# TravisWheelerLab/BATH

Hardware: AMD Instinct MI355X
Metric: DP Gcells/s + residues/s through bathsearch pipeline at 1/2/4/8 MI355X (higher is better)
Workload: dtype u8/i16 integer scores (SSV: exact binary16), f32 Forward

## Files before the change

### bath_amd/csrc/bath_kernels.hpp

```cpp
#pragma once
#include <climits>
#include <hip/hip_runtime.h>

#include <cstdint>

#include "bath_common.hpp"
#include "bath_hip.h"

namespace bath {

typedef short s16x2 __attribute__((ext_vector_type(2)));

template <int CTRL, int ROW_MASK = 0xf>
__device__ __forceinline__ int dpp_i(int v, int old) { return __builtin_amdgcn_update_dpp(old, v, CTRL, ROW_MASK, 0xf, false); }
__device__ __forceinline__ int wave_shr1_i32(int v, int fill) { return dpp_i<0x138>(v, fill); }
__device__ __forceinline__ float wave_shr1_f32(float v, float fill) {
  return __builtin_bit_cast(float, __builtin_amdgcn_update_dpp(__builtin_bit_cast(int, fill), __builtin_bit_cast(int, v), 0x138, 0xf, 0xf, false));
}
__device__ __forceinline__ float wave_max_f32(float v) {
  const int ninf = (int)0xff800000;
#define BATH_FMAX_STEP(CTRL, MASK) v = fmaxf(v, __builtin_bit_cast(float, __builtin_amdgcn_update_dpp(ninf, __builtin_bit_cast(int, v), CTRL, MASK, 0xf, false)));
  BATH_FMAX_STEP(0x111, 0xf) BATH_FMAX_STEP(0x112, 0xf) BATH_FMAX_STEP(0x114, 0xf) BATH_FMAX_STEP(0x118, 0xf) BATH_FMAX_STEP(0x142, 0xa) BATH_FMAX_STEP(0x143, 0xc)
#undef BATH_FMAX_STEP
  return __builtin_bit_cast(float, __builtin_amdgcn_readlane(__builtin_bit_cast(int, v), 63));
// ... 158 lines not shown
    const s16x2 xBv = __builtin_bit_cast(s16x2, bh);
    const s16x2 wrap = __builtin_bit_cast(s16x2, __builtin_amdgcn_alignbit(__builtin_bit_cast(unsigned, reg[NR - 1]), 0u, 16));
    s16x2 xE = zero, xE2 = zero;
#pragma unroll
    for (int g = NR / 4 - 1; g >= 0; g--) {
      const ssv_i4 inc = row[g];
      const int r = 4 * g;
      const s16x2 v3 = ssv_add(msv_pkmax(reg[r + 2], xBv), inc.w);
      const s16x2 v2 = ssv_add(msv_pkmax(reg[r + 1], xBv), inc.z);
      const s16x2 v1 = ssv_add(msv_pkmax(reg[r], xBv), inc.y);
      const s16x2 v0 = ssv_add(msv_pkmax((r > 0) ? reg[r - 1] : wrap, xBv), inc.x);
      reg[r + 3] = v3; reg[r + 2] = v2; reg[r + 1] = v1; reg[r] = v0;
      xE = ssv_max3(xE, v3, v2);
      xE2 = ssv_max3(xE2, v1, v0);
    }
    const h16x2 e1 = __builtin_bit_cast(h16x2, xE), e2 = __builtin_bit_cast(h16x2, xE2);
    int xEi = (int)(fmaxf(fmaxf((float)e1.x, (float)e1.y), fmaxf((float)e2.x, (float)e2.y)) * 2048.0f);
    if (xEi + c.bias >= 255) over = true;
    xEi = max(xEi - c.tec, 0);
    xJ = max(xJ, xEi);
    xB = max(max(c.base, xJ) - tjbm, 0);
  }
  *overflow = over;
  return xJ;
}
__device__ __forceinline__ float msv_lane_score(int xJ, int tjb, const MsvConsts &c) {
  float r = ((float)(xJ - tjb) - (float)c.base);
  r /= c.scale_b;
  return (float)((double)r - 3.0);
}

struct WindowRec { int32_t cand, n, k, length; float score; };

__device__ __forceinline__ float bias_forward(const uint8_t *s, int L, int M, const float *e , float p1) {
  const float L1 = (float)M / 8.0f;
  const float t00 = p1, t01 = 1.0f - p1, t10 = 1.0f / (L1 + 1.0f), t11 = L1 / (L1 + 1.0f);
  float logsc = 0.0f;
  if (L <= 0) return logsc;
  int x = min((int)s[0], 28);
  float d0 = e[2 * x] * 0.999f, d1 = e[2 * x + 1] * 0.001f;
  float mx = fmaxf(fmaxf(d0, 0.0f), d1);
  d0 /= mx; d1 /= mx;
  logsc += (float)log((double)mx);
  auto step = [&](int xx) {
    float n0 = 0.0f + d0 * t00; n0 = n0 + d1 * t10; n0 *= e[2 * xx];
    float n1 = 0.0f + d0 * t01; n1 = n1 + d1 * t11; n1 *= e[2 * xx + 1];
    mx = fmaxf(fmaxf(n0, 0.0f), n1);
    d0 = n0 / mx; d1 = n1 / mx;
    logsc += (float)log((double)mx);
  };
  int i = 1;
  uint32_t wnext = (i + 4 <= L) ? *reinterpret_cast<const uint32_t *>(s + i) : 0u;
  for (; i + 4 <= L; i += 4) {
    const uint32_t w = wnext;
    if (i + 8 <= L) wnext = *reinterpret_cast<const uint32_t *>(s + i + 4);
#pragma unroll
    for (int j = 0; j < 4; j++) step(min((int)((w >> (8 * j)) & 0xffu), 28));
  }
  for (; i < L; i++) step(min((int)s[i], 28));
  float end = 0.0f + d0 * 1.0f; end = end + d1 * 1.0f;
  logsc += (float)log((double)end);
  return logsc;
}

}
```

### bath_amd/csrc/bath_pipeline.hip

```cpp
#include <algorithm>
#include <cmath>
#include <cstring>
#include <cstdlib>
#include <map>
#include <thread>

#include "bath_common.hpp"
#include "bath_kernels.hpp"
#include "bath_launch.hpp"
#include "host_model.hpp"

using namespace bath;

namespace bath {

static const double kLog2 = 0.69314718055994529;

enum { FLAG_VIT_RUN = 1, FLAG_HAS_WIN = 2 };

struct Counters {
  int cand_count, todo_msv, todo_vit, todo_ssvb, todo_vit2, todo_fwd, win_count, overflow;
  int todo_lb, pad_;
  unsigned long long n_orfs, orf_res;
  unsigned long long n_past_msv, n_past_bias, n_past_vit, n_past_fwd;
// ... 295 lines not shown
  for (int k = k_start; k <= k_end; k++) {
    const float lo = ((float)base_b - (float)ssv_scores[(size_t)k * kKp + x]) / scale_b;
    acc += bgf[x] * expf(lo);
  }
  return acc;
}
__device__ void local_compo_finish(float *compo , const float *bgf, float *eo );
__device__ void local_compo_eo(const uint8_t *ssv_scores, int M, int base_b, float scale_b, const float *bgf, int k_start, int k_end, float *eo ) {
  float compo[20];
  for (int x = 0; x < 20; x++) compo[x] = local_compo_x(ssv_scores, M, base_b, scale_b, bgf, k_start, k_end, x);
  local_compo_finish(compo, bgf, eo);
}
__device__ void local_compo_finish(float *compo, const float *bgf, float *eo) {
  float sum = 0.f, cc = 0.f;
  for (int x = 0; x < 20; x++) { const float y = compo[x] - cc; const float t = sum + y; cc = (t - sum) - y; sum = t; }
  if (sum != 0.0f) for (int x = 0; x < 20; x++) compo[x] /= sum;
  else for (int x = 0; x < 20; x++) compo[x] = 1.0f / 20.0f;
  for (int x = 0; x < 20; x++) { eo[2 * x] = bgf[x] / bgf[x]; eo[2 * x + 1] = compo[x] / bgf[x]; }
  eo[2 * 20] = eo[2 * 20 + 1] = 1.0f; eo[2 * 27] = eo[2 * 27 + 1] = 1.0f; eo[2 * 28] = eo[2 * 28 + 1] = 1.0f;
  const int mem[6][2] = {{2, 11}, {7, 9}, {3, 13}, {8, 8}, {1, 1}, {-1, -1}};
  for (int dx = 0; dx < 6; dx++) {
    float n0 = 0.f, n1 = 0.f, den = 0.f;
    if (dx == 5) { for (int y = 0; y < 20; y++) { n0 += bgf[y]; n1 += compo[y]; den += bgf[y]; } }
    else {
      const int a = min(mem[dx][0], mem[dx][1]), b = max(mem[dx][0], mem[dx][1]);
      n0 += bgf[a]; n1 += compo[a]; den += bgf[a];
      if (b != a) { n0 += bgf[b]; n1 += compo[b]; den += bgf[b]; }
    }
    eo[2 * (21 + dx)] = den > 0.f ? n0 / den : 0.f;
    eo[2 * (21 + dx) + 1] = den > 0.f ? n1 / den : 0.f;
  }
}

__global__ void post_vit_kernel(Cand cand, int cand_cap, Counters *__restrict__ ctr, Params p, int32_t *__restrict__ todo_lb, int32_t *__restrict__ todo_fwd) {
  const int ncand = min(ctr->cand_count, cand_cap);
  for (int c = blockIdx.x * blockDim.x + threadIdx.x; c < ncand; c += gridDim.x * blockDim.x) {
    if (cand.stage[c] != 2) continue;
    const int L = cand.len[c];
    if (cand.flags[c] & FLAG_VIT_RUN) {
      const float seqsc = (float)((double)(cand.vfsc[c] - cand.filtersc[c]) / kLog2);
      const double P = d_gumbel_surv(seqsc, p.evparam[2], p.evparam[3]);
      cand.P[c] = P;
      if (P > p.F2) { cand.kminmax[2 * c] = 1 << 30; cand.kminmax[2 * c + 1] = 0; continue; }
    }
    atomicAdd(&ctr->n_past_vit, 1ull); atomicAdd(&ctr->pos_past_vit, (unsigned long long)L * 3ull);
    if (p.do_bias && cand.kminmax[2 * c] <= cand.kminmax[2 * c + 1]) {
      cand.flags[c] |= FLAG_HAS_WIN;
      todo_lb[atomicAdd(&ctr->todo_lb, 1)] = c;
      continue;
    }
    cand.stage[c] = 3;
    todo_fwd[atomicAdd(&ctr->todo_fwd, 1)] = c; atomicAdd(&ctr->res_fwd, (unsigned long long)L);
  }
}

__global__ void compo_terms_kernel(const float *__restrict__ bgf, int base_b, float scale_b, float *__restrict__ terms ) {
  const int x = blockIdx.x, sc = threadIdx.x;
  const float lo = ((float)base_b - (float)sc) / scale_b;
  terms[x * 256 + sc] = bgf[x] * expf(lo);
}

__global__ __launch_bounds__(64) void local_compo_kernel(Cand cand, const Counters *__restrict__ ctr, int M, const uint8_t *__restrict__ ssv_scores,
                                                         const float *__restrict__ terms, const int32_t *__restrict__ todo_lb, float *__restrict__ compo_out ) {
  const int lane = threadIdx.x, g = lane / 20, x = lane % 20;
  const int ntodo = ctr->todo_lb;
  for (int base = blockIdx.x * 3; base < ntodo; base += gridDim.x * 3) {
    const int job = base + g;
    if (g >= 3 || job >= ntodo) continue;
    const int c = todo_lb[job];
    int k_start = cand.kminmax[2 * c], k_end = cand.kminmax[2 * c + 1];
    const int k_len = k_end - k_start + 1;
    if (k_len < 20) { k_start -= (20 - k_len) / 2; k_end += (20 - k_len) / 2; }
    k_start = max(1, k_start); k_end = min(M, k_end);
    const float *tx = terms + x * 256;
    float acc = 0.0f;
    for (int k = k_start; k <= k_end; k++) acc += tx[ssv_scores[(size_t)k * kKp + x]];
    compo_out[(size_t)job * 20 + x] = acc;
  }
}

__global__ __launch_bounds__(64) void post_vit_local_kernel(Cand cand, Counters *__restrict__ ctr, Params p, const uint8_t *__restrict__ pool, int M,
                                                            const float *__restrict__ bgf, const float *__restrict__ compo_in,
                                                            const float *__restrict__ p1_tab, const float *__restrict__ lt1_tab, const float *__restrict__ lt2_tab,
                                                            const int32_t *__restrict__ todo_lb, int32_t *__restrict__ todo_vit2, int32_t *__restrict__ todo_fwd) {
  __shared__ float s_eo[64][kKp * 2 + 1];
  const int ntodo = ctr->todo_lb;
  for (int job = blockIdx.x * blockDim.x + threadIdx.x; job < ntodo; job += gridDim.x * blockDim.x) {
    const int c = todo_lb[job];
    const int L = cand.len[c];
    const float usc = cand.usc[c];
    float filtersc = cand.filtersc[c];
    const float vfsc = (cand.flags[c] & FLAG_VIT_RUN) ? cand.vfsc[c] : -INFINITY;
    float compo[20];
    for (int y = 0; y < 20; y++) compo[y] = compo_in[(size_t)job * 20 + y];
    float *eo = s_eo[threadIdx.x];
    local_compo_finish(compo, bgf, eo);
    float lf = bias_forward(pool + cand.off[c], L, M, eo, p1_tab[L]);
    lf = (lf + lt1_tab[L]) + lt2_tab[L];
    bool to_fwd = true;
    if (lf > filtersc) {
      filtersc = lf;
      cand.filtersc[c] = filtersc;
      if (vfsc == -INFINITY) {
        const float seqsc = (float)((double)(usc - filtersc) / kLog2);
        const double P = d_gumbel_surv(seqsc, p.evparam[0], p.evparam[1]);
        cand.P[c] = P;
        if (P > p.F2) { cand.stage[c] = 5; todo_vit2[atomicAdd(&ctr->todo_vit2, 1)] = c; atomicAdd(&ctr->res_vit, (unsigned long long)L); to_fwd = false; }
      } else {
        const float seqsc = (float)((double)(vfsc - filtersc) / kLog2);
        const double P = d_gumbel_surv(seqsc, p.evparam[2], p.evparam[3]);
        cand.P[c] = P;
        if (P > p.F2) to_fwd = false;
      }
    }
    if (to_fwd) { cand.stage[c] = 3; todo_fwd[atomicAdd(&ctr->todo_fwd, 1)] = c; atomicAdd(&ctr->res_fwd, (unsigned long long)L); }
  }
}

__global__ void post_vit2_kernel(Cand cand, Counters *__restrict__ ctr, Params p, const int32_t *__restrict__ todo_vit2, int32_t *__restrict__ todo_fwd) {
  const int ntodo = ctr->todo_vit2;
  for (int job = blockIdx.x * blockDim.x + threadIdx.x; job < ntodo; job += gridDim.x * blockDim.x) {
    const int c = todo_vit2[job];
    const float seqsc = (float)((double)(cand.vfsc[c] - cand.filtersc[c]) / kLog2);
    const double P = d_gumbel_surv(seqsc, p.evparam[2], p.evparam[3]);
    cand.P[c] = P;
    if (P > p.F2) { cand.stage[c] = 2; continue; }
    cand.stage[c] = 3;
    todo_fwd[atomicAdd(&ctr->todo_fwd, 1)] = c; atomicAdd(&ctr->res_fwd, (unsigned long long)cand.len[c]);
  }
}

__global__ void final_kernel(Cand cand, Counters *__restrict__ ctr, Params p, const int32_t *__restrict__ todo_fwd) {
  const int ntodo = ctr->todo_fwd;
  for (int job = blockIdx.x * blockDim.x + threadIdx.x; job < ntodo; job += gridDim.x * blockDim.x) {
    const int c = todo_fwd[job];
    const float seqsc = (float)((double)(cand.fwdsc[c] - cand.filtersc[c]) / kLog2);
    const double P = d_exp_surv(seqsc, p.evparam[4], p.evparam[5]);
    cand.P[c] = P;
    if (P > (p.fs_pipe ? p.F4 : p.F3)) continue;
    cand.stage[c] = 4;
    atomicAdd(&ctr->n_past_fwd, 1ull);
    if (!p.fs_pipe) atomicAdd(&ctr->pos_past_fwd, (unsigned long long)cand.len[c] * 3ull);
  }
}

__global__ void copy_count_kernel(const int *src, int64_t *dst) { *dst = *src; }

}
// ... 133 lines not shown
}

static int cascade_model_ok(bath_hip_ctx *ctx, const bath_hip_oprofile *om) {
  if (om->M <= kCascadeMaxNodes) return BATH_OK;
  ctx->set_error("the filter cascade supports models up to " + std::to_string(kCascadeMaxNodes) + " nodes (this one has " + std::to_string(om->M) + ")");
  return BATH_EINVAL;
}

static int launch_ssv_bath(bath_hip_ctx *ctx, hipStream_t stream, const bath_hip_oprofile *om, const Cand &cand, Counters *ctr, const int32_t *todo, const uint8_t *pool,
                           const uint8_t *ssv_scores, const MsvConsts &mc, double invP, WindowRec *wins, int win_cap);

static int run_filters(bath_hip_ctx *ctx, const bath_hip_oprofile *om, const bath_hip_seqs *dna,
                       const bath_pipeline_params *prm, bath_pipeline_stats *stats,
                       const bath_orf_result **results, int64_t *n_results, FilterState *state) {
  if (!ctx || !om || !dna || !prm) return BATH_EINVAL;
  if (cascade_model_ok(ctx, om) != BATH_OK) return BATH_EINVAL;
  BATH_HIP_TRY(ctx, hipSetDevice(ctx->device));
  if (n_results) *n_results = 0;
  if (results) *results = nullptr;
  if (stats) std::memset(stats, 0, sizeof *stats);
  const int64_t nwin = dna->n;
  if (nwin == 0) return BATH_OK;
  const int M = om->M;
  const int max_orf = dna->maxlen / 3 + 1;
  int st = om->ensure_len_tables(max_orf);
  if (st != BATH_OK) return st;

  OrfTablesDev tt{};
  if (prm->strands < 0 || prm->strands > 2 || prm->initiator < 0 || prm->initiator > 2) { ctx->set_error("bath_pipeline_params: strands / initiator out of range"); return BATH_EINVAL; }
  if ((st = orf_tables_upload(ctx, prm->ncbi_table, &tt, prm->initiator)) != BATH_OK) return st;
  if ((st = ensure_emit_table(ctx, om, prm->F1, max_orf)) != BATH_OK) return st;
  DevBuf &b_tabs = ctx->scratch[8], &b_work = ctx->scratch[9];
  const size_t ssv_bytes = (size_t)(M + 1) * kKp;
  const size_t tabs_bytes = 8192 + ssv_bytes + 256 + 20 * 4 + 256;
  if (tabs_bytes > b_tabs.cap) ctx->tabs_uid = 0;
  BATH_HIP_TRY(ctx, b_tabs.reserve(tabs_bytes));
  char *tp = b_tabs.as<char>();
  const int16_t *d_emit = om->d_emit;
  uint8_t *d_ssvsc = reinterpret_cast<uint8_t *>(tp); tp += (ssv_bytes + 255) / 256 * 256;
  float *d_bgf = reinterpret_cast<float *>(tp);
  if (ctx->tabs_uid != om->uid || ctx->tabs_ptr != b_tabs.p) {
    std::vector<uint8_t> ssv_scores(ssv_bytes, 0);
    bath_hip_oprofile_get_ssv_scores(om, ssv_scores.data());
    BATH_HIP_TRY(ctx, hipMemcpyAsync(d_ssvsc, ssv_scores.data(), ssv_scores.size(), hipMemcpyHostToDevice, ctx->stream));
    BATH_HIP_TRY(ctx, hipMemcpyAsync(d_bgf, kAminoBg, 20 * sizeof(float), hipMemcpyHostToDevice, ctx->stream));
    BATH_HIP_TRY(ctx, hipStreamSynchronize(ctx->stream));
    ctx->tabs_uid = om->uid; ctx->tabs_ptr = b_tabs.p;
  }

  Params P{};
  P.F1 = prm->F1; P.F2 = prm->F2; P.F3 = prm->F3; P.F4 = prm->F4;
  P.do_bias = prm->do_biasfilter; P.fs_pipe = prm->fs_pipe; P.minlen = prm->min_orf_len;
  std::memcpy(P.evparam, om->evparam, sizeof P.evparam);
  const MsvConsts mc = msv_consts(om);
  const double invP_f1 = gumbel_invsurv(prm->F1, om->evparam[0], om->evparam[1]);
  VitWindowArgs wa{};
  wa.invP_vit = (double)(float)gumbel_invsurv(prm->F2, om->evparam[2], om->evparam[3]);
  wa.invP_msv = (double)(float)gumbel_invsurv(prm->F2, om->evparam[0], om->evparam[1]);

  if (dna->cache_minlen != prm->min_orf_len) {
    int64_t nres_c = 0, max_orfs_c = 0;
    for (int64_t i = 0; i < nwin; i++) {
      const int n = dna->h_len[i];
      if (n < 15) continue;
      nres_c += 2 * (int64_t)(n - (dna->h_context.empty() ? 0 : dna->h_context[(size_t)i]));
      max_orfs_c += 6 * (int64_t)((n / 3 + 1) / (prm->min_orf_len + 1) + 1);
    }
    dna->cache_minlen = prm->min_orf_len; dna->cache_nres = nres_c; dna->cache_max_orfs = max_orfs_c;
  }
  const int64_t nres = prm->strands == BATH_STRAND_BOTH ? dna->cache_nres : dna->cache_nres / 2;
  const int64_t max_orfs = dna->cache_max_orfs;
  if (max_orfs >= (int64_t)INT32_MAX) { ctx->set_error("DNA block too large for one pipeline call (ORF list indices are 32-bit): split it"); return BATH_EINVAL; }
  int64_t cap = std::max<int64_t>(4096, (int64_t)((double)max_orfs * std::min(1.0, prm->F1 * 4.0 + 0.01)));
  cap = std::min<int64_t>(cap, std::max<int64_t>(max_orfs, 4096));

  if ((st = orf_tiles_ensure(ctx, dna)) != BATH_OK) return st;
  const size_t nent = (size_t)dna->ntiles * 6;
  DevBuf &b_aa = ctx->scratch[24], &b_slots = ctx->scratch[25], &b_orfs = ctx->scratch[26], &b_misc = ctx->scratch[27];
// ... 64 lines not shown
                       om->ssv_row_bytes, om->lt.d_tjb, mc, P, W.pool, M, f1t, W.todo_vit, W.todo_ssvb);                                      \
    launched = true;                                                                                                                        \
  }
      BATH_MSV_LANE_NR(BATH_MSV_STAGE_CASE)
#undef BATH_MSV_STAGE_CASE
      if (!launched) { ctx->set_error("MSV stage kernel: no tile shape for this model length"); return BATH_EINVAL; }
      BATH_HIP_TRY(ctx, hipGetLastError());
      BATH_HIP_TRY(ctx, hipEventRecord(ev[e++], ctx->stream));
      BATH_HIP_TRY(ctx, hipEventRecord(ev[e++], ctx->stream));
    } else {
      hipLaunchKernelGGL(classify_kernel, dim3(dec_blocks), dim3(256), 0, ctx->stream, W.cand, W.cand_cap, W.ctr, om->lt.d_tjb, mc, W.todo_msv);
      BATH_HIP_TRY(ctx, hipGetLastError());
      if ((st = launch_msv_wave(ctx, om, cv, W.todo_msv, cap, W.cand.usc, W.cand.msv_status, &W.ctr->todo_msv, !few_msv)) != BATH_OK) return st;
      BATH_HIP_TRY(ctx, hipEventRecord(ev[e++], ctx->stream));
      hipLaunchKernelGGL(f1_bias_kernel, dim3(dec_blocks), dim3(256), 0, ctx->stream, W.cand, W.cand_cap, W.ctr, P, W.pool, M, f1t, W.todo_vit, W.todo_ssvb);
      BATH_HIP_TRY(ctx, hipGetLastError());
      BATH_HIP_TRY(ctx, hipEventRecord(ev[e++], ctx->stream));
    }
    wa.d_filtersc = W.cand.filtersc; wa.d_ssv_scores = d_ssvsc; wa.d_wins = W.wins; wa.d_win_count = &W.ctr->win_count; wa.win_cap = W.win_cap;
    wa.d_kminmax = W.cand.kminmax;
    auto launch_ssvb = [&](hipStream_t stream) -> int {
      return launch_ssv_bath(ctx, stream, om, W.cand, W.ctr, W.todo_ssvb, W.pool, d_ssvsc, mc, invP_f1, W.wins, W.win_cap);
    };
    bool ssvb_done = false;
    if (vit_lane_supported(om) && !few_cands) {
      if ((st = launch_vit_sorted(ctx, om, cv, W.todo_vit, cap, &W.ctr->todo_vit, W.cand.len, W.len_bins, W.todo_sorted, W.cand.vfsc, W.cand.vit_status, &wa,
                                  launch_ssvb)) != BATH_OK) return st;
      ssvb_done = true;
    } else if ((st = launch_vit_wave(ctx, om, cv, W.todo_vit, cap, W.cand.vfsc, W.cand.vit_status, &wa, &W.ctr->todo_vit)) != BATH_OK) return st;
    BATH_HIP_TRY(ctx, hipEventRecord(ev[e++], ctx->stream));
    if (!ssvb_done && (st = launch_ssvb(ctx->stream)) != BATH_OK) return st;
    BATH_HIP_TRY(ctx, hipGetLastError());
    BATH_HIP_TRY(ctx, hipEventRecord(ev[e++], ctx->stream));
    hipLaunchKernelGGL(post_vit_kernel, dim3(dec_blocks), dim3(256), 0, ctx->stream, W.cand, W.cand_cap, W.ctr, P, W.todo_msv , W.todo_fwd);
    if (P.do_bias) {
      DevBuf &b_compo = ctx->scratch[36];
      BATH_HIP_TRY(ctx, b_compo.reserve((size_t)20 * 256 * 4 + (size_t)W.cand_cap * 20 * 4 + 256));
      float *d_terms = b_compo.as<float>(), *d_compo = d_terms + 20 * 256;
      hipLaunchKernelGGL(compo_terms_kernel, dim3(20), dim3(256), 0, ctx->stream, d_bgf, (int)om->base_b, om->scale_b, d_terms);
      hipLaunchKernelGGL(local_compo_kernel, dim3(16384), dim3(64), 0, ctx->stream, W.cand, W.ctr, M, d_ssvsc, d_terms, W.todo_msv, d_compo);
      hipLaunchKernelGGL(post_vit_local_kernel, dim3(std::max(1, dec_blocks)), dim3(64), 0, ctx->stream, W.cand, W.ctr, P, W.pool, M, d_bgf, d_compo,
                         om->lt.d_p1, om->lt.d_lt1, om->lt.d_lt2, W.todo_msv, W.todo_vit2, W.todo_fwd);
    }
    BATH_HIP_TRY(ctx, hipGetLastError());
    if ((st = launch_vit_wave(ctx, om, cv, W.todo_vit2, cap, W.cand.vfsc, W.cand.vit_status, nullptr, &W.ctr->todo_vit2)) != BATH_OK) return st;
    hipLaunchKernelGGL(post_vit2_kernel, dim3(64), dim3(256), 0, ctx->stream, W.cand, W.ctr, P, W.todo_vit2, W.todo_fwd);
    BATH_HIP_TRY(ctx, hipGetLastError());
    BATH_HIP_TRY(ctx, hipEventRecord(ev[e++], ctx->stream));
    ctx->fwd_rows_kept = nullptr; ctx->fwd_rows_off = nullptr;
    float *d_keep = nullptr; int64_t *d_keep_off = nullptr;
    if (ctx->keep_fwd_rows) {
      constexpr int64_t kKeepFloats = (int64_t)8 << 20;
      DevBuf &b_rows = ctx->scratch[38], &b_roff = ctx->scratch[39];
      BATH_HIP_TRY(ctx, b_rows.reserve((size_t)kKeepFloats * sizeof(float) + 64)); BATH_HIP_TRY(ctx, b_roff.reserve((size_t)cap * sizeof(int64_t) + 64));
      d_keep = b_rows.as<float>(); d_keep_off = b_roff.as<int64_t>();
      hipLaunchKernelGGL(fwd_keep_offsets_kernel, dim3(1), dim3(64), 0, ctx->stream, W.todo_fwd, &W.ctr->todo_fwd, W.cand.len, d_keep_off, kKeepFloats);
      BATH_HIP_TRY(ctx, hipGetLastError());
    }
    if ((st = launch_fwd_wave(ctx, om, cv, W.todo_fwd, cap, W.cand.fwdsc, W.cand.fwd_status, &W.ctr->todo_fwd, d_keep, d_keep_off)) != BATH_OK) return st;
    if (d_keep) { ctx->fwd_rows_kept = d_keep; ctx->fwd_rows_off = d_keep_off; }
    hipLaunchKernelGGL(final_kernel, dim3(dec_blocks), dim3(256), 0, ctx->stream, W.cand, W.ctr, P, W.todo_fwd);
    BATH_HIP_TRY(ctx, hipGetLastError());
    BATH_HIP_TRY(ctx, hipEventRecord(ev[e++], ctx->stream));

    BATH_HIP_TRY(ctx, hipMemcpyAsync(&hc, W.ctr, sizeof(Counters), hipMemcpyDeviceToHost, ctx->stream));
    BATH_HIP_TRY(ctx, hipStreamSynchronize(ctx->stream));
    if (hc.overflow || hc.cand_count > cap || hc.win_count > W.win_cap) {
      if (attempt >= 4) { ctx->set_error("candidate / window buffers overflowed repeatedly"); return BATH_EMEM; }
      if (hc.overflow || hc.cand_count > cap) cap = std::max<int64_t>(cap * 2, (int64_t)hc.cand_count + 1024);
      if (hc.win_count > W.win_cap) win_need = hc.win_count + hc.win_count / 4 + 1024;
      continue;
    }
    static const char *names[] = {"translate_orfs", "ssv_f1", "classify_msv", "f1_bias", "viterbi_windows", "ssv_windows", "post_vit", "forward_final"};
    const int64_t launches[] = {4, 1, msv_stage ? 1 : 2, msv_stage ? 0 : 1, 4, 1, 3, 2};
    ctx->timings.clear();
    for (int i = 0; i + 1 < e; i++) {
      float ms = 0.f;
      BATH_HIP_TRY(ctx, hipEventElapsedTime(&ms, ev[i], ev[i + 1]));
      ctx->timings.push_back(StageTiming{names[i], ms, launches[i]});
    }
    break;
  }

  if (stats) {
    stats->nres = nres; stats->n_orfs = (int64_t)hc.n_orfs;
    stats->n_past_msv = (int64_t)hc.n_past_msv; stats->n_past_bias = (int64_t)hc.n_past_bias;
    stats->n_past_vit = (int64_t)hc.n_past_vit; stats->n_past_fwd = (int64_t)hc.n_past_fwd;
    stats->pos_past_msv = (int64_t)hc.pos_past_msv; stats->pos_past_bias = (int64_t)hc.pos_past_bias;
    stats->pos_past_vit = (int64_t)hc.pos_past_vit; stats->pos_past_fwd = (int64_t)hc.pos_past_fwd;
    stats->cells_msv = (int64_t)(hc.orf_res - hc.res_seen) * M; stats->cells_vit = (int64_t)hc.res_vit * M; stats->cells_fwd = (int64_t)hc.res_fwd * M;
  }

  if (results) {
    bath_orf_result *d_rec = nullptr;
    int64_t nrec = 0;
    if (dna->n > (int64_t)UINT32_MAX || dna->maxlen / 3 >= (1 << 28)) { ctx->set_error("block too large for the ORF records' sort key (2^32 windows, 805 Mnt per window)"); return BATH_ERANGE; }
    if ((st = build_orf_records(ctx, W.cand, hc.cand_count, dna->is_part ? dna->first_window : 0, &d_rec, &nrec)) != BATH_OK) return st;
    ctx->d_records = d_rec; ctx->n_records = nrec;
    if (!dna->is_part) {
      BATH_HIP_TRY(ctx, ctx->results_pinned.reserve((size_t)std::max<int64_t>(nrec, 1) * sizeof(bath_orf_result)));
      if (nrec > 0) BATH_HIP_TRY(ctx, hipMemcpyAsync(ctx->results_pinned.p, d_rec, (size_t)nrec * sizeof(bath_orf_result), hipMemcpyDeviceToHost, ctx->stream));
      BATH_HIP_TRY(ctx, hipStreamSynchronize(ctx->stream));
      *results = ctx->results_pinned.as<bath_orf_result>();
    } else *results = nullptr;
    if (n_results) *n_results = nrec;
  } else if (n_results) *n_results = (int64_t)hc.n_past_msv;
  if (state) { state->W = W; state->hc = hc; state->d_ssvsc = d_ssvsc; state->d_bgf = d_bgf; state->tt = tt; }
// ... 617 lines not shown
```

### bath_amd/csrc/bath_viterbi.hip

```cpp
#include <algorithm>
#include <cstdlib>
#include <functional>

#include "bath_common.hpp"
#include "bath_kernels.hpp"
#include "bath_launch.hpp"

using namespace bath;

namespace bath {

__device__ __forceinline__ s16x2 pk_adds(s16x2 a, s16x2 b) { return __builtin_elementwise_add_sat(a, b); }
__device__ __forceinline__ s16x2 pk_max(s16x2 a, s16x2 b) { return __builtin_elementwise_max(a, b); }
__device__ __forceinline__ s16x2 as_s2(unsigned v) { return __builtin_bit_cast(s16x2, v); }
__device__ __forceinline__ unsigned as_u(s16x2 v) { return __builtin_bit_cast(unsigned, v); }

struct VitLaneTables {
  const int16_t *rw;
  int rw_pitch_bytes;
  const uint32_t *tw2;
  const int16_t *rank;
};

struct VitLaneConsts {
// ... 145 lines not shown
        }
      }
    }
  }
  if (live) {
    if (overflow) { sc[sid] = INFINITY; status[sid] = BATH_ERANGE; }
    else if (xC > -32768) {
      float r = (float)xC + (float)xw_move - (float)c.base_w;
      r /= c.scale_w;
      r = (float)((double)r - 3.0);
      sc[sid] = r; status[sid] = BATH_OK;
    } else { sc[sid] = -INFINITY; status[sid] = BATH_OK; }
    if (do_win && kminmax) { kminmax[2 * sid] = kmin; kminmax[2 * sid + 1] = kmax; }
  }
}

constexpr int kLenBins = 2048;
constexpr int kVitLongTarget = 128;
__device__ __forceinline__ void len_block_range(int n, int &lo, int &hi) {
  const int per = (n + (int)gridDim.x - 1) / (int)gridDim.x;
  lo = min(n, (int)blockIdx.x * per); hi = min(n, lo + per);
}
__global__ __launch_bounds__(256) void len_hist_kernel(const int32_t *__restrict__ todo, const int *__restrict__ ntodo_dev, const int32_t *__restrict__ len,
                                                       int *__restrict__ hist) {
  __shared__ int s_cnt[kLenBins];
  for (int i = threadIdx.x; i < kLenBins; i += blockDim.x) s_cnt[i] = 0;
  __syncthreads();
  int lo, hi;
  len_block_range(*ntodo_dev, lo, hi);
  for (int j = lo + threadIdx.x; j < hi; j += blockDim.x) atomicAdd(&s_cnt[min(len[todo[j]], kLenBins - 1)], 1);
  __syncthreads();
  for (int i = threadIdx.x; i < kLenBins; i += blockDim.x) if (s_cnt[i]) atomicAdd(&hist[i], s_cnt[i]);
}
__global__ void len_scan_kernel(int *__restrict__ hist ) {
  __shared__ int tmp[kLenBins];
  for (int i = threadIdx.x; i < kLenBins; i += blockDim.x) tmp[i] = hist[i];
  __syncthreads();
  if (threadIdx.x == 0) {
    int run = 0;
    for (int b = kLenBins - 1; b >= 0; b--) { const int cnt = tmp[b]; tmp[b] = run; run += cnt; }
  }
  __syncthreads();
  for (int i = threadIdx.x; i < kLenBins; i += blockDim.x) hist[i] = tmp[i];
}
__global__ __launch_bounds__(256) void len_scatter_kernel(const int32_t *__restrict__ todo, const int *__restrict__ ntodo_dev, const int32_t *__restrict__ len,
                                                          int *__restrict__ cursor, int32_t *__restrict__ sorted) {
  __shared__ int s_cnt[kLenBins];
  for (int i = threadIdx.x; i < kLenBins; i += blockDim.x) s_cnt[i] = 0;
  __syncthreads();
  int lo, hi;
  len_block_range(*ntodo_dev, lo, hi);
  for (int j = lo + threadIdx.x; j < hi; j += blockDim.x) atomicAdd(&s_cnt[min(len[todo[j]], kLenBins - 1)], 1);
  __syncthreads();
  for (int i = threadIdx.x; i < kLenBins; i += blockDim.x) { const int c = s_cnt[i]; if (c) s_cnt[i] = atomicAdd(&cursor[i], c); }
  __syncthreads();
  for (int j = lo + threadIdx.x; j < hi; j += blockDim.x) {
    const int cnd = todo[j];
    sorted[atomicAdd(&s_cnt[min(len[cnd], kLenBins - 1)], 1)] = cnd;
  }
}

int vit_lane_supported(const bath_hip_oprofile *om) { return om->vit_NR > 0; }

const int *len_sort_count_longer(const int *d_bins, int T) { return d_bins + std::min(T + 1, kLenBins - 1); }

int launch_len_sort(bath_hip_ctx *ctx, const int32_t *d_todo, const int *d_ntodo, const int32_t *d_len, int *d_bins, int32_t *d_sorted) {
  BATH_HIP_TRY(ctx, hipMemsetAsync(d_bins, 0, kLenBins * sizeof(int), ctx->stream));
  hipLaunchKernelGGL(len_hist_kernel, dim3(256), dim3(256), 0, ctx->stream, d_todo, d_ntodo, d_len, d_bins);
  hipLaunchKernelGGL(len_scan_kernel, dim3(1), dim3(256), 0, ctx->stream, d_bins);
  hipLaunchKernelGGL(len_scatter_kernel, dim3(256), dim3(256), 0, ctx->stream, d_todo, d_ntodo, d_len, d_bins, d_sorted);
  BATH_HIP_TRY(ctx, hipGetLastError());
  return BATH_OK;
}

int launch_vit_lane(bath_hip_ctx *ctx, const bath_hip_oprofile *om, SeqView v, const int32_t *d_todo, int64_t ntodo, const int *ntodo_dev,
                    float *d_sc, int32_t *d_status, const VitWindowArgs *wa, const int *skip_dev) {
// ... 65 lines not shown
```

Baseline: 204.2 billion.

## Add fused post-Viterbi bias stage kernel and parallelize length scan

Adds a single-kernel post-Viterbi path that compacts the F2 survivors per block, computes local composition and the bias forward chain in LDS, and makes the routing decision in place. It is gated behind BATH_HIP_POST_VIT_SPLIT=0, so the split three-kernel path stays the default. The default path does get three changes: the compo-terms table moves to one-time table setup, the local composition sum is unrolled 8-way, and the serial single-thread histogram scan is replaced by a parallel wave scan. The fused kernel does its bias work on only one wave per block, which could leave the GPU underused.

```diff
diff --git a/bath_amd/csrc/bath_kernels.hpp b/bath_amd/csrc/bath_kernels.hpp
--- a/bath_amd/csrc/bath_kernels.hpp
+++ b/bath_amd/csrc/bath_kernels.hpp
@@ -214,34 +214,44 @@
 
 struct WindowRec { int32_t cand, n, k, length; float score; };
 
+struct BiasChain {
+  float t00, t01, t10, t11, d0, d1;
+  __device__ __forceinline__ BiasChain(int M, float p1) : d0(0.0f), d1(0.0f) {
+    const float L1 = (float)M / 8.0f;
+    t00 = p1; t01 = 1.0f - p1; t10 = 1.0f / (L1 + 1.0f); t11 = L1 / (L1 + 1.0f);
+  }
+  __device__ __forceinline__ float first(const float *e , int x) {
+    d0 = e[2 * x] * 0.999f; d1 = e[2 * x + 1] * 0.001f;
+    const float mx = fmaxf(fmaxf(d0, 0.0f), d1);
+    d0 /= mx; d1 /= mx;
+    return mx;
+  }
+  __device__ __forceinline__ float step(const float *e, int x) {
+    float n0 = 0.0f + d0 * t00; n0 = n0 + d1 * t10; n0 *= e[2 * x];
+    float n1 = 0.0f + d0 * t01; n1 = n1 + d1 * t11; n1 *= e[2 * x + 1];
+    const float mx = fmaxf(fmaxf(n0, 0.0f), n1);
+    d0 = n0 / mx; d1 = n1 / mx;
+    return mx;
+  }
+  __device__ __forceinline__ float end() const { float r = 0.0f + d0 * 1.0f; r = r + d1 * 1.0f; return r; }
+};
+__device__ __forceinline__ float bias_log(float mx) { return (float)log((double)mx); }
+
 __device__ __forceinline__ float bias_forward(const uint8_t *s, int L, int M, const float *e , float p1) {
-  const float L1 = (float)M / 8.0f;
-  const float t00 = p1, t01 = 1.0f - p1, t10 = 1.0f / (L1 + 1.0f), t11 = L1 / (L1 + 1.0f);
+  BiasChain ch(M, p1);
   float logsc = 0.0f;
   if (L <= 0) return logsc;
-  int x = min((int)s[0], 28);
-  float d0 = e[2 * x] * 0.999f, d1 = e[2 * x + 1] * 0.001f;
-  float mx = fmaxf(fmaxf(d0, 0.0f), d1);
-  d0 /= mx; d1 /= mx;
-  logsc += (float)log((double)mx);
-  auto step = [&](int xx) {
-    float n0 = 0.0f + d0 * t00; n0 = n0 + d1 * t10; n0 *= e[2 * xx];
-    float n1 = 0.0f + d0 * t01; n1 = n1 + d1 * t11; n1 *= e[2 * xx + 1];
-    mx = fmaxf(fmaxf(n0, 0.0f), n1);
-    d0 = n0 / mx; d1 = n1 / mx;
-    logsc += (float)log((double)mx);
-  };
+  logsc += bias_log(ch.first(e, min((int)s[0], 28)));
   int i = 1;
   uint32_t wnext = (i + 4 <= L) ? *reinterpret_cast<const uint32_t *>(s + i) : 0u;
   for (; i + 4 <= L; i += 4) {
     const uint32_t w = wnext;
     if (i + 8 <= L) wnext = *reinterpret_cast<const uint32_t *>(s + i + 4);
 #pragma unroll
-    for (int j = 0; j < 4; j++) step(min((int)((w >> (8 * j)) & 0xffu), 28));
-  }
-  for (; i < L; i++) step(min((int)s[i], 28));
-  float end = 0.0f + d0 * 1.0f; end = end + d1 * 1.0f;
-  logsc += (float)log((double)end);
+    for (int j = 0; j < 4; j++) logsc += bias_log(ch.step(e, min((int)((w >> (8 * j)) & 0xffu), 28)));
+  }
+  for (; i < L; i++) logsc += bias_log(ch.step(e, min((int)s[i], 28)));
+  logsc += bias_log(ch.end());
   return logsc;
 }
 
diff --git a/bath_amd/csrc/bath_pipeline.hip b/bath_amd/csrc/bath_pipeline.hip
--- a/bath_amd/csrc/bath_pipeline.hip
+++ b/bath_amd/csrc/bath_pipeline.hip
@@ -351,32 +351,168 @@
   }
 }
 
-__global__ void post_vit_kernel(Cand cand, int cand_cap, Counters *__restrict__ ctr, Params p, int32_t *__restrict__ todo_lb, int32_t *__restrict__ todo_fwd) {
-  const int ncand = min(ctr->cand_count, cand_cap);
-  for (int c = blockIdx.x * blockDim.x + threadIdx.x; c < ncand; c += gridDim.x * blockDim.x) {
-    if (cand.stage[c] != 2) continue;
-    const int L = cand.len[c];
-    if (cand.flags[c] & FLAG_VIT_RUN) {
-      const float seqsc = (float)((double)(cand.vfsc[c] - cand.filtersc[c]) / kLog2);
+__device__ __forceinline__ bool cand_f2(const Cand &cand, int c, Counters *__restrict__ ctr, const Params &p, int32_t *__restrict__ todo_fwd) {
+  if (cand.stage[c] != 2) return false;
+  const int L = cand.len[c];
+  if (cand.flags[c] & FLAG_VIT_RUN) {
+    const float seqsc = (float)((double)(cand.vfsc[c] - cand.filtersc[c]) / kLog2);
+    const double P = d_gumbel_surv(seqsc, p.evparam[2], p.evparam[3]);
+    cand.P[c] = P;
+    if (P > p.F2) { cand.kminmax[2 * c] = 1 << 30; cand.kminmax[2 * c + 1] = 0; return false; }
+  }
+  atomicAdd(&ctr->n_past_vit, 1ull); atomicAdd(&ctr->pos_past_vit, (unsigned long long)L * 3ull);
+  if (p.do_bias && cand.kminmax[2 * c] <= cand.kminmax[2 * c + 1]) { cand.flags[c] |= FLAG_HAS_WIN; return true; }
+  cand.stage[c] = 3;
+  todo_fwd[atomicAdd(&ctr->todo_fwd, 1)] = c; atomicAdd(&ctr->res_fwd, (unsigned long long)L);
+  return false;
+}
+
+__device__ __forceinline__ float local_compo_sum(int k_start, int k_end, int M, const uint8_t *__restrict__ ssv_scores, const float *__restrict__ terms, int x) {
+  const int k_len = k_end - k_start + 1;
+  if (k_len < 20) { k_start -= (20 - k_len) / 2; k_end += (20 - k_len) / 2; }
+  k_start = max(1, k_start); k_end = min(M, k_end);
+  const float *tx = terms + x * 256;
+  float acc = 0.0f;
+  int k = k_start;
+  for (; k + 8 <= k_end + 1; k += 8) {
+    float t[8];
+#pragma unroll
+    for (int u = 0; u < 8; u++) t[u] = tx[ssv_scores[(size_t)(k + u) * kKp + x]];
+#pragma unroll
+    for (int u = 0; u < 8; u++) acc += t[u];
+  }
+  for (; k <= k_end; k++) acc += tx[ssv_scores[(size_t)k * kKp + x]];
+  return acc;
+}
+
+__device__ __forceinline__ void cand_local_decide(const Cand &cand, int c, Counters *__restrict__ ctr, const Params &p, float lf,
+                                                  int32_t *__restrict__ todo_vit2, int32_t *__restrict__ todo_fwd) {
+  const int L = cand.len[c];
+  const float usc = cand.usc[c];
+  float filtersc = cand.filtersc[c];
+  const float vfsc = (cand.flags[c] & FLAG_VIT_RUN) ? cand.vfsc[c] : -INFINITY;
+  bool to_fwd = true;
+  if (lf > filtersc) {
+    filtersc = lf;
+    cand.filtersc[c] = filtersc;
+    if (vfsc == -INFINITY) {
+      const float seqsc = (float)((double)(usc - filtersc) / kLog2);
+      const double P = d_gumbel_surv(seqsc, p.evparam[0], p.evparam[1]);
+      cand.P[c] = P;
+      if (P > p.F2) { cand.stage[c] = 5; todo_vit2[atomicAdd(&ctr->todo_vit2, 1)] = c; atomicAdd(&ctr->res_vit, (unsigned long long)L); to_fwd = false; }
+    } else {
+      const float seqsc = (float)((double)(vfsc - filtersc) / kLog2);
       const double P = d_gumbel_surv(seqsc, p.evparam[2], p.evparam[3]);
       cand.P[c] = P;
-      if (P > p.F2) { cand.kminmax[2 * c] = 1 << 30; cand.kminmax[2 * c + 1] = 0; continue; }
-    }
-    atomicAdd(&ctr->n_past_vit, 1ull); atomicAdd(&ctr->pos_past_vit, (unsigned long long)L * 3ull);
-    if (p.do_bias && cand.kminmax[2 * c] <= cand.kminmax[2 * c + 1]) {
-      cand.flags[c] |= FLAG_HAS_WIN;
-      todo_lb[atomicAdd(&ctr->todo_lb, 1)] = c;
-      continue;
-    }
-    cand.stage[c] = 3;
-    todo_fwd[atomicAdd(&ctr->todo_fwd, 1)] = c; atomicAdd(&ctr->res_fwd, (unsigned long long)L);
-  }
+      if (P > p.F2) to_fwd = false;
+    }
+  }
+  if (to_fwd) { cand.stage[c] = 3; todo_fwd[atomicAdd(&ctr->todo_fwd, 1)] = c; atomicAdd(&ctr->res_fwd, (unsigned long long)L); }
 }
 
 __global__ void compo_terms_kernel(const float *__restrict__ bgf, int base_b, float scale_b, float *__restrict__ terms ) {
   const int x = blockIdx.x, sc = threadIdx.x;
   const float lo = ((float)base_b - (float)sc) / scale_b;
   terms[x * 256 + sc] = bgf[x] * expf(lo);
+}
+
+constexpr int kBiasChunk = 128;
+constexpr int kStageGroup = 16;
+struct PostVitLds {
+  int cid[256];
+  int wn[4];
+  int64_t off[kStageGroup];
+  int len[kStageGroup];
+  float eo[kStageGroup][kKp * 2 + 1];
+  float compo[kStageGroup][20];
+  float mx[kStageGroup][kBiasChunk + 1];
+  uint32_t res[kStageGroup][kBiasChunk / 4 + 1];
+};
+__device__ __forceinline__ void wave_lds_fence() { asm volatile("s_waitcnt lgkmcnt(0)" ::: "memory"); }
+
+__global__ __launch_bounds__(256) void post_vit_stage_kernel(Cand cand, int cand_cap, Counters *__restrict__ ctr, Params p, const uint8_t *__restrict__ pool, int M,
+                                                             const uint8_t *__restrict__ ssv_scores, const float *__restrict__ terms, const float *__restrict__ bgf,
+                                                             const float *__restrict__ p1_tab, const float *__restrict__ lt1_tab, const float *__restrict__ lt2_tab,
+                                                             int32_t *__restrict__ todo_vit2, int32_t *__restrict__ todo_fwd) {
+  __shared__ PostVitLds S;
+  const int ncand = min(ctr->cand_count, cand_cap);
+  if ((int64_t)blockIdx.x * blockDim.x >= ncand) return;
+  const int lane = threadIdx.x & 63, wv = threadIdx.x >> 6;
+  const int64_t job = (int64_t)blockIdx.x * blockDim.x + threadIdx.x;
+  const bool listed = job < ncand && cand_f2(cand, (int)job, ctr, p, todo_fwd);
+  const unsigned long long mask = __ballot(listed);
+  if (lane == 0) S.wn[wv] = __popcll(mask);
+  __syncthreads();
+  int base = 0, nlisted = 0;
+#pragma unroll
+  for (int u = 0; u < 4; u++) { base += u < wv ? S.wn[u] : 0; nlisted += S.wn[u]; }
+  if (listed) S.cid[base + __popcll(mask & ((1ull << lane) - 1ull))] = (int)job;
+  __threadfence();
+  __syncthreads();
+  if (wv != 0) return;
+  for (int g0 = 0; g0 < nlisted; g0 += kStageGroup) {
+    const int ng = min(kStageGroup, nlisted - g0);
+    const bool own = lane < ng;
+    const int c = own ? S.cid[g0 + lane] : 0;
+    const int L = own ? cand.len[c] : 0;
+    const uint8_t *s = pool + (own ? cand.off[c] : 0);
+    if (own) { S.len[lane] = L; S.off[lane] = cand.off[c]; }
+    for (int r0 = 0; r0 < ng; r0 += 3) {
+      const int gl = lane / 20, x = lane % 20, g = r0 + gl;
+      if (gl < 3 && g < ng) {
+        const int cg = S.cid[g0 + g];
+        S.compo[g][x] = local_compo_sum(cand.kminmax[2 * cg], cand.kminmax[2 * cg + 1], M, ssv_scores, terms, x);
+      }
+    }
+    wave_lds_fence();
+    const float *e = S.eo[own ? lane : 0];
+    if (own) local_compo_finish(S.compo[lane], bgf, S.eo[lane]);
+    wave_lds_fence();
+    BiasChain ch(M, p1_tab[L]);
+    float logsc = 0.0f;
+    if (L > 0) logsc += bias_log(ch.first(e, min((int)s[0], 28)));
+    const int Lmax = wave_max_i32(L);
+    for (int i0 = 1; i0 < Lmax; i0 += kBiasChunk) {
+      const int n = min(kBiasChunk, L - i0);
+      for (int g = 0; g < ng; g++) {
+        const int ngr = min(kBiasChunk, S.len[g] - i0);
+        const uint8_t *sg = pool + S.off[g] + i0;
+        uint8_t *dst = reinterpret_cast<uint8_t *>(S.res[g]);
+        for (int j = lane; j < ngr; j += 64) dst[j] = (uint8_t)min((int)sg[j], 28);
+      }
+      wave_lds_fence();
+      if (own) {
+        float *mx = S.mx[lane];
+        int j = 0;
+        for (; j + 4 <= n; j += 4) {
+          const uint32_t w = S.res[lane][j >> 2];
+#pragma unroll
+          for (int u = 0; u < 4; u++) mx[j + u] = ch.step(e, (int)((w >> (8 * u)) & 0xffu));
+        }
+        for (; j < n; j++) mx[j] = ch.step(e, (int)((S.res[lane][j >> 2] >> (8 * (j & 3))) & 0xffu));
+      }
+      wave_lds_fence();
+      for (int g = 0; g < ng; g++) {
+        const int ngr = min(kBiasChunk, S.len[g] - i0);
+        for (int j = lane; j < ngr; j += 64) S.mx[g][j] = bias_log(S.mx[g][j]);
+      }
+      wave_lds_fence();
+      if (own) for (int j = 0; j < n; j++) logsc += S.mx[lane][j];
+      wave_lds_fence();
+    }
+    if (own) {
+      if (L > 0) logsc += bias_log(ch.end());
+      const float lf = (logsc + lt1_tab[L]) + lt2_tab[L];
+      cand_local_decide(cand, c, ctr, p, lf, todo_vit2, todo_fwd);
+    }
+    wave_lds_fence();
+  }
+}
+
+__global__ void post_vit_kernel(Cand cand, int cand_cap, Counters *__restrict__ ctr, Params p, int32_t *__restrict__ todo_lb, int32_t *__restrict__ todo_fwd) {
+  const int ncand = min(ctr->cand_count, cand_cap);
+  for (int c = blockIdx.x * blockDim.x + threadIdx.x; c < ncand; c += gridDim.x * blockDim.x)
+    if (cand_f2(cand, c, ctr, p, todo_fwd)) todo_lb[atomicAdd(&ctr->todo_lb, 1)] = c;
 }
 
 __global__ __launch_bounds__(64) void local_compo_kernel(Cand cand, const Counters *__restrict__ ctr, int M, const uint8_t *__restrict__ ssv_scores,
@@ -387,14 +523,7 @@
     const int job = base + g;
     if (g >= 3 || job >= ntodo) continue;
     const int c = todo_lb[job];
-    int k_start = cand.kminmax[2 * c], k_end = cand.kminmax[2 * c + 1];
-    const int k_len = k_end - k_start + 1;
-    if (k_len < 20) { k_start -= (20 - k_len) / 2; k_end += (20 - k_len) / 2; }
-    k_start = max(1, k_start); k_end = min(M, k_end);
-    const float *tx = terms + x * 256;
-    float acc = 0.0f;
-    for (int k = k_start; k <= k_end; k++) acc += tx[ssv_scores[(size_t)k * kKp + x]];
-    compo_out[(size_t)job * 20 + x] = acc;
+    compo_out[(size_t)job * 20 + x] = local_compo_sum(cand.kminmax[2 * c], cand.kminmax[2 * c + 1], M, ssv_scores, terms, x);
   }
 }
 
@@ -407,32 +536,13 @@
   for (int job = blockIdx.x * blockDim.x + threadIdx.x; job < ntodo; job += gridDim.x * blockDim.x) {
     const int c = todo_lb[job];
     const int L = cand.len[c];
-    const float usc = cand.usc[c];
-    float filtersc = cand.filtersc[c];
-    const float vfsc = (cand.flags[c] & FLAG_VIT_RUN) ? cand.vfsc[c] : -INFINITY;
     float compo[20];
     for (int y = 0; y < 20; y++) compo[y] = compo_in[(size_t)job * 20 + y];
     float *eo = s_eo[threadIdx.x];
     local_compo_finish(compo, bgf, eo);
     float lf = bias_forward(pool + cand.off[c], L, M, eo, p1_tab[L]);
     lf = (lf + lt1_tab[L]) + lt2_tab[L];
-    bool to_fwd = true;
-    if (lf > filtersc) {
-      filtersc = lf;
-      cand.filtersc[c] = filtersc;
-      if (vfsc == -INFINITY) {
-        const float seqsc = (float)((double)(usc - filtersc) / kLog2);
-        const double P = d_gumbel_surv(seqsc, p.evparam[0], p.evparam[1]);
-        cand.P[c] = P;
-        if (P > p.F2) { cand.stage[c] = 5; todo_vit2[atomicAdd(&ctr->todo_vit2, 1)] = c; atomicAdd(&ctr->res_vit, (unsigned long long)L); to_fwd = false; }
-      } else {
-        const float seqsc = (float)((double)(vfsc - filtersc) / kLog2);
-        const double P = d_gumbel_surv(seqsc, p.evparam[2], p.evparam[3]);
-        cand.P[c] = P;
-        if (P > p.F2) to_fwd = false;
-      }
-    }
-    if (to_fwd) { cand.stage[c] = 3; todo_fwd[atomicAdd(&ctr->todo_fwd, 1)] = c; atomicAdd(&ctr->res_fwd, (unsigned long long)L); }
+    cand_local_decide(cand, c, ctr, p, lf, todo_vit2, todo_fwd);
   }
 }
 
@@ -632,18 +742,21 @@
   if ((st = ensure_emit_table(ctx, om, prm->F1, max_orf)) != BATH_OK) return st;
   DevBuf &b_tabs = ctx->scratch[8], &b_work = ctx->scratch[9];
   const size_t ssv_bytes = (size_t)(M + 1) * kKp;
-  const size_t tabs_bytes = 8192 + ssv_bytes + 256 + 20 * 4 + 256;
+  const size_t tabs_bytes = 8192 + ssv_bytes + 256 + 256 + 20 * 256 * 4 + 256;
   if (tabs_bytes > b_tabs.cap) ctx->tabs_uid = 0;
   BATH_HIP_TRY(ctx, b_tabs.reserve(tabs_bytes));
   char *tp = b_tabs.as<char>();
   const int16_t *d_emit = om->d_emit;
   uint8_t *d_ssvsc = reinterpret_cast<uint8_t *>(tp); tp += (ssv_bytes + 255) / 256 * 256;
-  float *d_bgf = reinterpret_cast<float *>(tp);
+  float *d_bgf = reinterpret_cast<float *>(tp); tp += 256;
+  float *d_terms = reinterpret_cast<float *>(tp);
   if (ctx->tabs_uid != om->uid || ctx->tabs_ptr != b_tabs.p) {
     std::vector<uint8_t> ssv_scores(ssv_bytes, 0);
     bath_hip_oprofile_get_ssv_scores(om, ssv_scores.data());
     BATH_HIP_TRY(ctx, hipMemcpyAsync(d_ssvsc, ssv_scores.data(), ssv_scores.size(), hipMemcpyHostToDevice, ctx->stream));
     BATH_HIP_TRY(ctx, hipMemcpyAsync(d_bgf, kAminoBg, 20 * sizeof(float), hipMemcpyHostToDevice, ctx->stream));
+    hipLaunchKernelGGL(compo_terms_kernel, dim3(20), dim3(256), 0, ctx->stream, d_bgf, (int)om->base_b, om->scale_b, d_terms);
+    BATH_HIP_TRY(ctx, hipGetLastError());
     BATH_HIP_TRY(ctx, hipStreamSynchronize(ctx->stream));
     ctx->tabs_uid = om->uid; ctx->tabs_ptr = b_tabs.p;
   }
@@ -774,15 +887,20 @@
     if (!ssvb_done && (st = launch_ssvb(ctx->stream)) != BATH_OK) return st;
     BATH_HIP_TRY(ctx, hipGetLastError());
     BATH_HIP_TRY(ctx, hipEventRecord(ev[e++], ctx->stream));
-    hipLaunchKernelGGL(post_vit_kernel, dim3(dec_blocks), dim3(256), 0, ctx->stream, W.cand, W.cand_cap, W.ctr, P, W.todo_msv , W.todo_fwd);
-    if (P.do_bias) {
-      DevBuf &b_compo = ctx->scratch[36];
-      BATH_HIP_TRY(ctx, b_compo.reserve((size_t)20 * 256 * 4 + (size_t)W.cand_cap * 20 * 4 + 256));
-      float *d_terms = b_compo.as<float>(), *d_compo = d_terms + 20 * 256;
-      hipLaunchKernelGGL(compo_terms_kernel, dim3(20), dim3(256), 0, ctx->stream, d_bgf, (int)om->base_b, om->scale_b, d_terms);
-      hipLaunchKernelGGL(local_compo_kernel, dim3(16384), dim3(64), 0, ctx->stream, W.cand, W.ctr, M, d_ssvsc, d_terms, W.todo_msv, d_compo);
-      hipLaunchKernelGGL(post_vit_local_kernel, dim3(std::max(1, dec_blocks)), dim3(64), 0, ctx->stream, W.cand, W.ctr, P, W.pool, M, d_bgf, d_compo,
-                         om->lt.d_p1, om->lt.d_lt1, om->lt.d_lt2, W.todo_msv, W.todo_vit2, W.todo_fwd);
+    static const bool post_vit_split = [] { const char *e = std::getenv("BATH_HIP_POST_VIT_SPLIT"); return !e || std::atoi(e) != 0; }();
+    if (!post_vit_split) {
+      hipLaunchKernelGGL(post_vit_stage_kernel, dim3((unsigned)((W.cand_cap + 255) / 256)), dim3(256), 0, ctx->stream, W.cand, W.cand_cap, W.ctr, P, W.pool, M,
+                         d_ssvsc, d_terms, d_bgf, om->lt.d_p1, om->lt.d_lt1, om->lt.d_lt2, W.todo_vit2, W.todo_fwd);
+    } else {
+      hipLaunchKernelGGL(post_vit_kernel, dim3(dec_blocks), dim3(256), 0, ctx->stream, W.cand, W.cand_cap, W.ctr, P, W.todo_msv , W.todo_fwd);
+      if (P.do_bias) {
+        DevBuf &b_compo = ctx->scratch[36];
+        BATH_HIP_TRY(ctx, b_compo.reserve((size_t)W.cand_cap * 20 * 4 + 256));
+        float *d_compo = b_compo.as<float>();
+        hipLaunchKernelGGL(local_compo_kernel, dim3(16384), dim3(64), 0, ctx->stream, W.cand, W.ctr, M, d_ssvsc, d_terms, W.todo_msv, d_compo);
+        hipLaunchKernelGGL(post_vit_local_kernel, dim3(std::max(1, dec_blocks)), dim3(64), 0, ctx->stream, W.cand, W.ctr, P, W.pool, M, d_bgf, d_compo,
+                           om->lt.d_p1, om->lt.d_lt1, om->lt.d_lt2, W.todo_msv, W.todo_vit2, W.todo_fwd);
+      }
     }
     BATH_HIP_TRY(ctx, hipGetLastError());
     if ((st = launch_vit_wave(ctx, om, cv, W.todo_vit2, cap, W.cand.vfsc, W.cand.vit_status, nullptr, &W.ctr->todo_vit2)) != BATH_OK) return st;
@@ -814,7 +932,7 @@
       continue;
     }
     static const char *names[] = {"translate_orfs", "ssv_f1", "classify_msv", "f1_bias", "viterbi_windows", "ssv_windows", "post_vit", "forward_final"};
-    const int64_t launches[] = {4, 1, msv_stage ? 1 : 2, msv_stage ? 0 : 1, 4, 1, 3, 2};
+    const int64_t launches[] = {4, 1, msv_stage ? 1 : 2, msv_stage ? 0 : 1, 4, 1, !post_vit_split ? 3 : P.do_bias ? 5 : 3, 2};
     ctx->timings.clear();
     for (int i = 0; i + 1 < e; i++) {
       float ms = 0.f;
diff --git a/bath_amd/csrc/bath_viterbi.hip b/bath_amd/csrc/bath_viterbi.hip
--- a/bath_amd/csrc/bath_viterbi.hip
+++ b/bath_amd/csrc/bath_viterbi.hip
@@ -201,16 +201,23 @@
   __syncthreads();
   for (int i = threadIdx.x; i < kLenBins; i += blockDim.x) if (s_cnt[i]) atomicAdd(&hist[i], s_cnt[i]);
 }
-__global__ void len_scan_kernel(int *__restrict__ hist ) {
-  __shared__ int tmp[kLenBins];
-  for (int i = threadIdx.x; i < kLenBins; i += blockDim.x) tmp[i] = hist[i];
-  __syncthreads();
-  if (threadIdx.x == 0) {
-    int run = 0;
-    for (int b = kLenBins - 1; b >= 0; b--) { const int cnt = tmp[b]; tmp[b] = run; run += cnt; }
-  }
-  __syncthreads();
-  for (int i = threadIdx.x; i < kLenBins; i += blockDim.x) hist[i] = tmp[i];
+__global__ __launch_bounds__(256) void len_scan_kernel(int *__restrict__ hist ) {
+  constexpr int kPer = kLenBins / 256;
+  __shared__ int s_wsum[4];
+  const int tid = threadIdx.x, lane = tid & 63, wv = tid >> 6;
+  int c[kPer], sum = 0;
+#pragma unroll
+  for (int k = 0; k < kPer; k++) { c[k] = hist[kLenBins - 1 - (kPer * tid + k)]; sum += c[k]; }
+  int x = sum;
+#pragma unroll
+  for (int d = 1; d < 64; d <<= 1) { const int y = __shfl_up(x, d, 64); if (lane >= d) x += y; }
+  if (lane == 63) s_wsum[wv] = x;
+  __syncthreads();
+  int run = x - sum;
+#pragma unroll
+  for (int u = 0; u < 4; u++) run += u < wv ? s_wsum[u] : 0;
+#pragma unroll
+  for (int k = 0; k < kPer; k++) { hist[kLenBins - 1 - (kPer * tid + k)] = run; run += c[k]; }
 }
 __global__ __launch_bounds__(256) void len_scatter_kernel(const int32_t *__restrict__ todo, const int *__restrict__ ntodo_dev, const int32_t *__restrict__ len,
                                                           int *__restrict__ cursor, int32_t *__restrict__ sorted) {
```

New measurement: 204.1 billion. No clear change (-0.1%).
